# openMVG/openMVG

Measured on AMD Instinct MI355X. Metric: descriptor pairs/s (brute-force L2 2-NN + ratio matching), higher is better.
Workload: dtype i8 (int32 accumulate); 1 GPU; 1000 images x 2000 SIFT-like uint8x128 descriptors, exhaustive pairs (499500 image pairs, 499500 on rank 0), ratio 0.8; parallelism=pair-sharded x1, no collective

## Files before the change

openmvg_amd/csrc/mvgx_match.hip:

```cpp
#include <hip/hip_runtime.h>

#include <algorithm>
#include <atomic>
#include <climits>
#include <condition_variable>
#include <cstdint>
#include <cstdlib>
#include <cstring>
#include <functional>
#include <mutex>
#include <string>
#include <thread>
#include <vector>

#include "mvgx_common.h"

namespace {

using mvgx::set_error;

typedef int v4i __attribute__((ext_vector_type(4)));
typedef int v16i __attribute__((ext_vector_type(16)));

constexpr int kDim = 128;
constexpr int kTileRows = 32;
constexpr int kTileBytes = kTileRows * kDim;
constexpr int kWinTiles = 8;
constexpr int kWinRows = kWinTiles * kTileRows;
constexpr int kWaves = 4;
constexpr int kNQ = 4;
constexpr int kBlockQTiles = kWaves * kNQ;
constexpr int kRecQuads = 1 + kWaves;
constexpr int kStageBytes = kWinTiles * kTileBytes + kWinTiles * kTileRows * 4;
constexpr int kRPad = INT_MIN + 512;
constexpr int kCPad = -(1 << 27);
constexpr int kNegInit = -(1 << 28);
constexpr uint32_t kNoMatch = 0xFFFFFFFFu;
constexpr int kTailTiles = 16;

struct MatchParams {
  const int8_t* tiles;
  const int8_t* rows_slot;
  const int* rconst;
  const int* cinit;
  const int* qnorm;
  const uint32_t* perm;
  const uint32_t* rowpos;
  const uint8_t* rows_u8;
  const uint64_t* img_row_off;
  const uint32_t* img_tile_off;
  const uint32_t* img_n;
  const uint32_t* img_ntiles;
  const uint32_t* img_neven;
  const int8_t* qtiles;
  const int* qtnorm;
  const uint2* pairs;
  const uint2* work;
  const uint4* work8h;
  const uint4* work8;
  uint32_t n_work;
  uint32_t* best;
  int2* cd;
  uint32_t* count;
  uint32_t* errflag;
  uint32_t qstride;
  float ratio_sq;
};

__global__ __launch_bounds__(256) void row_norms_kernel(const uint8_t* __restrict__ rows,
                                                        const uint64_t* __restrict__ img_row_off,
                                                        const uint32_t* __restrict__ img_n, int* __restrict__ rownorm,
                                                        uint32_t* __restrict__ n_even) {
  const uint32_t img = blockIdx.y;
  const uint32_t n = img_n[img];
  const uint32_t r = blockIdx.x * blockDim.x + threadIdx.x;
  bool even = false;
  if (r < n) {
    const uint4* src = reinterpret_cast<const uint4*>(rows + (img_row_off[img] + r) * kDim);
    int nn = 0;
#pragma unroll
    for (int c = 0; c < 8; ++c) {
      uint4 v = src[c];
      const uint32_t w[4] = {v.x ^ 0x80808080u, v.y ^ 0x80808080u, v.z ^ 0x80808080u, v.w ^ 0x80808080u};
#pragma unroll
      for (int i = 0; i < 4; ++i) nn = __builtin_amdgcn_sdot4((int)w[i], (int)w[i], nn, false);
    }
    rownorm[img_row_off[img] + r] = nn;
    even = (nn & 1) == 0;
  }
  const unsigned long long m = __ballot(even);
  if ((threadIdx.x & 63) == 0 && m) atomicAdd(&n_even[img], (uint32_t)__popcll(m));
}

__device__ __host__ __forceinline__ int slot_row(int j, int h) { return (j >> 2) * 8 + h * 4 + (j & 3); }

__global__ __launch_bounds__(1024) void assign_slots_kernel(const uint64_t* __restrict__ img_row_off,
                                                            const uint32_t* __restrict__ img_tile_off,
                                                            const uint32_t* __restrict__ img_n,
                                                            const int* __restrict__ rownorm, uint32_t* __restrict__ rowpos,
                                                            uint32_t* __restrict__ perm, int* __restrict__ rconst,
                                                            int* __restrict__ cinit, int* __restrict__ qnorm) {
  __shared__ uint32_t s_cnt[16][2];
  __shared__ uint32_t s_base[2];
  const uint32_t img = blockIdx.x;
  const uint32_t n = img_n[img];
  const uint64_t row0 = img_row_off[img];
  const size_t slot0 = (size_t)img_tile_off[img] * kTileRows;
  const int lane = threadIdx.x & 63, wave = threadIdx.x >> 6;
  if (threadIdx.x < 2) s_base[threadIdx.x] = 0;
  __syncthreads();
  for (uint32_t c0 = 0; c0 < n; c0 += blockDim.x) {
    const uint32_t r = c0 + threadIdx.x;
    const bool valid = r < n;
    const int nn = valid ? rownorm[row0 + r] : 0;
    const int par = nn & 1;
    const unsigned long long m_even = __ballot(valid && par == 0), m_odd = __ballot(valid && par == 1);
    if (lane == 0) { s_cnt[wave][0] = (uint32_t)__popcll(m_even); s_cnt[wave][1] = (uint32_t)__popcll(m_odd); }
    __syncthreads();
    if (valid) {
      uint32_t rank = s_base[par];
      for (int w = 0; w < wave; ++w) rank += s_cnt[w][par];
      rank += (uint32_t)__popcll((par ? m_odd : m_even) & ((1ull << lane) - 1ull));
      const uint32_t t = rank >> 4;
      const uint32_t pos = t * kTileRows + (uint32_t)slot_row((int)(rank & 15u), par);
      rowpos[row0 + r] = pos;
      perm[slot0 + pos] = r;
      rconst[slot0 + pos] = -(nn << 8) - (int)((t % kWinTiles) * kTileRows + (pos & 31u));
      cinit[slot0 + pos] = -(nn >> 1);
      qnorm[slot0 + pos] = nn;
    }
    __syncthreads();
    if (threadIdx.x == 0) {
      uint32_t e = 0, o = 0;
      for (int w = 0; w < 16; ++w) { e += s_cnt[w][0]; o += s_cnt[w][1]; }
      s_base[0] += e; s_base[1] += o;
    }
    __syncthreads();
  }
}

__global__ __launch_bounds__(256) void build_tiles_kernel(const uint8_t* __restrict__ rows,
                                                          const uint64_t* __restrict__ img_row_off,
                                                          const uint32_t* __restrict__ img_tile_off,
                                                          const uint32_t* __restrict__ perm, int8_t* __restrict__ tiles,
                                                          int8_t* __restrict__ rows_slot) {
  const uint32_t img = blockIdx.y;
  const uint32_t ntiles_pad = img_tile_off[img + 1] - img_tile_off[img];
  const uint32_t t = blockIdx.x;
  if (t >= ntiles_pad) return;
  const uint32_t gt = img_tile_off[img] + t;
  const int c = threadIdx.x;
  const int s = c >> 6, lane = c & 63;
  const int m = lane & 31, h = lane >> 5;
  const uint32_t src_row = perm[(size_t)gt * kTileRows + m];
  uint4 v = make_uint4(0, 0, 0, 0);
  if (src_row != kNoMatch) {
    v = *reinterpret_cast<const uint4*>(rows + (img_row_off[img] + src_row) * kDim + (s * 2 + h) * 16);
    v.x ^= 0x80808080u; v.y ^= 0x80808080u; v.z ^= 0x80808080u; v.w ^= 0x80808080u;
  }
  *reinterpret_cast<uint4*>(tiles + (size_t)gt * kTileBytes + c * 16) = v;
  *reinterpret_cast<uint4*>(rows_slot + ((size_t)gt * kTileRows + m) * kDim + (s * 2 + h) * 16) = v;
}

__global__ __launch_bounds__(256) void build_qtiles_kernel(const uint8_t* __restrict__ rows,
                                                           const uint64_t* __restrict__ img_row_off,
                                                           const uint32_t* __restrict__ img_qtile_off,
                                                           const uint32_t* __restrict__ img_n,
                                                           const int* __restrict__ rownorm, int8_t* __restrict__ qtiles,
                                                           int* __restrict__ qtnorm) {
  const uint32_t img = blockIdx.y;
  const uint32_t t = blockIdx.x;
  if (t >= img_qtile_off[img + 1] - img_qtile_off[img]) return;
  const uint32_t gt = img_qtile_off[img] + t;
  const int c = threadIdx.x;
  const int s = c >> 6, lane = c & 63;
  const int m = lane & 31, h = lane >> 5;
  const uint32_t r = t * kTileRows + (uint32_t)m;
  const bool real = r < img_n[img];
  uint4 v = make_uint4(0, 0, 0, 0);
  if (real) {
    v = *reinterpret_cast<const uint4*>(rows + (img_row_off[img] + r) * kDim + (s * 2 + h) * 16);
    v.x ^= 0x80808080u; v.y ^= 0x80808080u; v.z ^= 0x80808080u; v.w ^= 0x80808080u;
  }
  *reinterpret_cast<uint4*>(qtiles + (size_t)gt * kTileBytes + c * 16) = v;
  if (c < kTileRows) qtnorm[(size_t)gt * kTileRows + m] = real ? rownorm[img_row_off[img] + r] : 0;
}

__global__ __launch_bounds__(256) void fill_i32_kernel(int* __restrict__ p, size_t n, int value) {
  const size_t i = (size_t)blockIdx.x * blockDim.x + threadIdx.x;
  if (i < n) p[i] = value;
}

__device__ __forceinline__ int med3i(int a, int b, int c) { return max(min(a, b), min(max(a, b), c)); }

__device__ __forceinline__ uint32_t xcd_remap(uint32_t b, uint32_t nwg) {
  const uint32_t q = nwg >> 3, r = nwg & 7u;
  const uint32_t xcd = b & 7u, pos = b >> 3;
  const uint32_t base = (xcd < r) ? xcd * (q + 1) : r * (q + 1) + (xcd - r) * q;
  return base + pos;
}

enum StageMode { kStageRegs = 1, kStageGlds = 2, kStageGldsAsm = 3 };


__device__ __forceinline__ void glds16_asm(const void* gsrc, unsigned lds_dst) {
  unsigned keep;
  asm volatile(
      "s_mov_b32 %0, m0\n\ts_mov_b32 m0, %2\n\ts_nop 0\n\tglobal_load_lds_dwordx4 %1, off\n\ts_mov_b32 m0, %0"
      : "=&s"(keep)
      : "v"(gsrc), "s"(lds_dst)
      : "memory");
}
__device__ __forceinline__ void glds4_asm(const void* gsrc, unsigned lds_dst) {
  unsigned keep;
  asm volatile(
      "s_mov_b32 %0, m0\n\ts_mov_b32 m0, %2\n\ts_nop 0\n\tglobal_load_lds_dword %1, off\n\ts_mov_b32 m0, %0"
      : "=&s"(keep)
      : "v"(gsrc), "s"(lds_dst)
      : "memory");
}
__device__ __forceinline__ void stage_window_glds_asm(char* buf, const int8_t* __restrict__ gtiles,
                                                      const int* __restrict__ grconst, int wave, int lane) {
  const unsigned lds0 = (unsigned)(size_t)(__attribute__((address_space(3))) char*)buf;
#pragma unroll
  for (int i = 0; i < kWinTiles; ++i) {
    const int off = i * kTileBytes + wave * 1024;
    glds16_asm(gtiles + off + lane * 16, __builtin_amdgcn_readfirstlane(lds0 + off));
  }
  glds4_asm(grconst + wave * 64 + lane, __builtin_amdgcn_readfirstlane(lds0 + kWinTiles * kTileBytes + wave * 256));
}

constexpr int kHalfTiles = kWinTiles / 2;
constexpr int kHalfStageBytes = kHalfTiles * kTileBytes + kHalfTiles * kTileRows * 4;
__device__ __forceinline__ void stage_half_glds_asm(char* buf, const int8_t* __restrict__ gtiles, const int* __restrict__ grconst, int wave, int lane) {
  const unsigned lds0 = (unsigned)(size_t)(__attribute__((address_space(3))) char*)buf;
#pragma unroll
  for (int i = 0; i < kHalfTiles; ++i) {
    const int off = i * kTileBytes + wave * 1024;
    glds16_asm(gtiles + off + lane * 16, __builtin_amdgcn_readfirstlane(lds0 + off));
  }
  if (wave < 2) glds4_asm(grconst + wave * 64 + lane, __builtin_amdgcn_readfirstlane(lds0 + kHalfTiles * kTileBytes + wave * 256));
}

__device__ __forceinline__ void stage_window_glds(char* buf, const int8_t* __restrict__ gtiles,
                                                  const int* __restrict__ grconst, int wave, int lane) {
#pragma unroll
  for (int i = 0; i < kWinTiles; ++i) {
    const int off = i * kTileBytes + wave * 1024;
    __builtin_amdgcn_global_load_lds((const void __attribute__((address_space(1)))*)(gtiles + off + lane * 16),
                                     (void __attribute__((address_space(3)))*)(buf + off), 16, 0, 0);
  }
  __builtin_amdgcn_global_load_lds(
      (const void __attribute__((address_space(1)))*)(grconst + wave * 64 + lane),
      (void __attribute__((address_space(3)))*)(buf + kWinTiles * kTileBytes + wave * 256), 4, 0, 0);
}

struct StageRegs {
  uint4 v[kWinTiles];
  int r;
};
__device__ __forceinline__ void stage_issue(StageRegs& sr, const int8_t* __restrict__ gtiles,
                                            const int* __restrict__ grconst, int wave, int lane) {
#pragma unroll
  for (int i = 0; i < kWinTiles; ++i)
    sr.v[i] = *reinterpret_cast<const uint4*>(gtiles + i * kTileBytes + wave * 1024 + lane * 16);
  sr.r = grconst[wave * 64 + lane];
}
__device__ __forceinline__ void stage_commit(char* buf, const StageRegs& sr, int wave, int lane) {
#pragma unroll
  for (int i = 0; i < kWinTiles; ++i)
    *reinterpret_cast<uint4*>(buf + i * kTileBytes + wave * 1024 + lane * 16) = sr.v[i];
  *reinterpret_cast<int*>(buf + kWinTiles * kTileBytes + wave * 256 + lane * 4) = sr.r;
}

struct Item32 {
  uint32_t pair, tileI0, tileJ0, ntJpad, qt0;
  int ntI, nwin;
};
__device__ __forceinline__ Item32 load_item32(const MatchParams& p, int wave, int lane, v4i (&b)[kNQ][4]) {
  const uint32_t w = xcd_remap(blockIdx.x, gridDim.x);
  const uint2 wk = p.work[w];
  const uint2 ij = p.pairs[wk.x];
  const uint32_t I = ij.x, J = ij.y;
  Item32 it;
  it.pair = wk.x;
  it.tileI0 = p.img_tile_off[I]; it.tileJ0 = p.img_tile_off[J];
  it.ntJpad = p.img_tile_off[J + 1] - it.tileJ0;
  it.ntI = (int)p.img_ntiles[I];
  it.nwin = (it.ntI + kWinTiles - 1) / kWinTiles;
  it.qt0 = wk.y + (uint32_t)wave * kNQ;
  const int8_t* qsrc = p.tiles + (size_t)(it.tileJ0 + it.qt0) * kTileBytes + lane * 16;
#pragma unroll
  for (int n = 0; n < kNQ; ++n)
#pragma unroll
    for (int s = 0; s < 4; ++s) b[n][s] = *reinterpret_cast<const v4i*>(qsrc + n * kTileBytes + s * 1024);
  return it;
}
__device__ __forceinline__ void pin_fragments32(v4i (&b)[kNQ][4]) {
#pragma unroll
  for (int n = 0; n < kNQ; ++n)
#pragma unroll
    for (int s = 0; s < 4; ++s) asm volatile("" : "+v"(b[n][s]));
}
template <int kMode>
__device__ __forceinline__ void stage_first(char* smem, StageRegs& sr, const int8_t* __restrict__ gI, const int* __restrict__ gC, int wave, int lane) {
  if constexpr (kMode == kStageGlds) {
    stage_window_glds(smem, gI, gC, wave, lane);
  } else if constexpr (kMode == kStageGldsAsm) {
    stage_window_glds_asm(smem, gI, gC, wave, lane);
  } else {
    stage_issue(sr, gI, gC, wave, lane);
    stage_commit(smem, sr, wave, lane);
  }
}
template <int kMode>
__device__ __forceinline__ void stage_next(char* nbuf, StageRegs& sr, const int8_t* __restrict__ gI, const int* __restrict__ gC, int win, int nwin,
                                           int wave, int lane) {
  if constexpr (kMode == kStageRegs) {
    const int wn = (win + 1 < nwin) ? win + 1 : win;
    stage_issue(sr, gI + (size_t)wn * kWinTiles * kTileBytes, gC + wn * kWinRows, wave, lane);
  } else if (win + 1 < nwin) {
    const int8_t* gt = gI + (size_t)(win + 1) * kWinTiles * kTileBytes;
    const int* gc = gC + (win + 1) * kWinRows;
    if constexpr (kMode == kStageGlds) stage_window_glds(nbuf, gt, gc, wave, lane);
    else stage_window_glds_asm(nbuf, gt, gc, wave, lane);
  }
}

template <int kMode>
__global__ __launch_bounds__(256, 2) void l2_top2_ratio_kernel(MatchParams p) {
  extern __shared__ __attribute__((aligned(16))) char smem[];

  const int lane = threadIdx.x & 63;
  const int wave = __builtin_amdgcn_readfirstlane(threadIdx.x >> 6);
  const int h = lane >> 5;

  v4i b[kNQ][4];
  const Item32 it = load_item32(p, wave, lane, b);
  const uint32_t tileI0 = it.tileI0, tileJ0 = it.tileJ0, ntJpad = it.ntJpad, qt0 = it.qt0;
  const int ntI = it.ntI, nwin = it.nwin;

  const int8_t* gI = p.tiles + (size_t)tileI0 * kTileBytes;
  const int* gR = p.rconst + (size_t)tileI0 * kTileRows;

  int G1[kNQ], G2[kNQ], Gi[kNQ];
#pragma unroll
  for (int n = 0; n < kNQ; ++n) { G1[n] = INT_MAX; G2[n] = INT_MAX; Gi[n] = 0; }

  StageRegs sr;
  stage_first<kMode>(smem, sr, gI, gR, wave, lane);
  pin_fragments32(b);

  for (int win = 0; win < nwin; ++win) {
    if constexpr (kMode == kStageGldsAsm) asm volatile("s_waitcnt vmcnt(0)" ::: "memory");
    __syncthreads();
    char* buf = smem + (win & 1) * kStageBytes;
    char* nbuf = smem + ((win + 1) & 1) * kStageBytes;
    stage_next<kMode>(nbuf, sr, gI, gR, win, nwin, wave, lane);

    int T1[kNQ], T2[kNQ];
#pragma unroll
    for (int n = 0; n < kNQ; ++n) { T1[n] = INT_MIN; T2[n] = INT_MIN; }

    const int nt = min(kWinTiles, ntI - win * kWinTiles);
    for (int t = 0; t < nt; ++t) {
      const char* tb = buf + t * kTileBytes + lane * 16;
      v4i a[4];
#pragma unroll
      for (int s = 0; s < 4; ++s) a[s] = *reinterpret_cast<const v4i*>(tb + s * 1024);
      const char* rb = buf + kWinTiles * kTileBytes + t * (kTileRows * 4) + h * 16;
      int R[16];
#pragma unroll
      for (int g = 0; g < 4; ++g) {
        const int4 rv = *reinterpret_cast<const int4*>(rb + g * 32);
        R[g * 4 + 0] = rv.x; R[g * 4 + 1] = rv.y; R[g * 4 + 2] = rv.z; R[g * 4 + 3] = rv.w;
      }
#pragma unroll
      for (int n = 0; n < kNQ; ++n) {
        v16i acc = {0, 0, 0, 0, 0, 0, 0, 0, 0, 0, 0, 0, 0, 0, 0, 0};
#pragma unroll
        for (int s = 0; s < 4; ++s) acc = __builtin_amdgcn_mfma_i32_32x32x32_i8(a[s], b[n][s], acc, 0, 0, 0);
        int t1 = T1[n], t2 = T2[n];
#pragma unroll
        for (int r = 0; r < 16; ++r) {
          const int T = (int)((unsigned)acc[r] << 9) + R[r];
          t2 = med3i(t1, t2, T);
          t1 = max(t1, T);
        }
        T1[n] = t1; T2[n] = t2;
      }
    }
    if constexpr (kMode == kStageRegs) stage_commit(nbuf, sr, wave, lane);
#pragma unroll
    for (int n = 0; n < kNQ; ++n) {
      const int k1 = -T1[n], k2 = -T2[n];
      const int wd1 = k1 >> 8, widx = (k1 & 255) + win * kWinRows, wd2 = k2 >> 8;
      const bool better = wd1 < G1[n];
      const int g2 = better ? min(G1[n], wd2) : min(G2[n], wd1);
      Gi[n] = better ? widx : Gi[n];
      G1[n] = better ? wd1 : G1[n];
      G2[n] = g2;
    }
  }

#pragma unroll
  for (int n = 0; n < kNQ; ++n) {
    const int P1 = __shfl_xor(G1[n], 32), P2 = __shfl_xor(G2[n], 32), Pi = __shfl_xor(Gi[n], 32);
    const bool better = P1 < G1[n];
    const int g2 = better ? min(G1[n], P2) : min(G2[n], P1);
    Gi[n] = better ? Pi : Gi[n];
    G1[n] = better ? P1 : G1[n];
    G2[n] = g2;
  }

#pragma unroll
  for (int n = 0; n < kNQ; ++n) {
    const uint32_t q = (qt0 + n) * kTileRows + (lane & 31);
    const bool inb = (lane < 32) && (qt0 + n < ntJpad);
    bool ok = false;
    if (inb) {
      const bool valid = p.perm[(size_t)tileJ0 * kTileRows + q] != kNoMatch;
      const int nq = p.qnorm[(size_t)tileJ0 * kTileRows + q];
      const int d0 = G1[n] + nq, d1 = G2[n] + nq;
      ok = valid && (__int2float_rn(d0) < __fmul_rn(p.ratio_sq, __int2float_rn(d1)));
      p.best[(size_t)it.pair * p.qstride + q] = ok ? p.perm[(size_t)tileI0 * kTileRows + (uint32_t)Gi[n]] : kNoMatch;
    }
    const unsigned long long m = __ballot(ok);
    if (lane == 0 && m) atomicAdd(&p.count[it.pair], (uint32_t)__popcll(m));
  }
}

__device__ __forceinline__ int max3i(int a, int b, int c) { return max(max(a, b), c); }

__device__ __forceinline__ void fold_window_max(int v, int& Q1, int& Q2, int& Qg, int win) {
  const bool better = v > Q1;
  Q2 = better ? Q1 : max(Q2, v);
  Qg = better ? win : Qg;
  Q1 = better ? v : Q1;
}
template <int kClasses>
__device__ __forceinline__ void fold_window(int (&TW)[kClasses], int (&TP)[kClasses], int& Q1, int& Q2, int& Qg, int win) {
  int v = TW[0];
#pragma unroll
  for (int c = 1; c < kClasses; ++c) v = max(v, TW[c]);
#pragma unroll
  for (int c = 0; c < kClasses; ++c) { TP[c] = max(TP[c], TW[c]); TW[c] = kNegInit; }
  fold_window_max(v, Q1, Q2, Qg, win);
}

enum FilterEpilogue { kEpiFold = 0, kEpiFoldOneCv = 1, kEpiPerChain = 2 };

template <int kMode, int kEpi = kEpiFold>
__global__ __launch_bounds__(256, 2) void l2_filter_kernel(MatchParams p) {
  extern __shared__ __attribute__((aligned(16))) char smem[];

  const int lane = threadIdx.x & 63;
  const int wave = __builtin_amdgcn_readfirstlane(threadIdx.x >> 6);
  const int h = lane >> 5;

  v4i b[kNQ][4];
  const Item32 it = load_item32(p, wave, lane, b);
  const uint32_t tileI0 = it.tileI0, tileJ0 = it.tileJ0, ntJpad = it.ntJpad, qt0 = it.qt0;
  const int ntI = it.ntI, nwin = it.nwin;

  const int8_t* gI = p.tiles + (size_t)tileI0 * kTileBytes;
  const int* gC = p.cinit + (size_t)tileI0 * kTileRows;

  constexpr bool kFold = kEpi != kEpiPerChain;
  constexpr bool kOneCv = kEpi == kEpiFoldOneCv;
  int TP[kNQ][8];
  int TW[kNQ][8];
  int Q1[kNQ], Q2[kNQ], Qg[kNQ];
#pragma unroll
  for (int n = 0; n < kNQ; ++n) {
#pragma unroll
    for (int s = 0; s < 8; ++s) { TP[n][s] = kNegInit; TW[n][s] = kNegInit; }
    Q1[n] = kNegInit; Q2[n] = kNegInit; Qg[n] = 0;
  }

  StageRegs sr;
  stage_first<kMode>(smem, sr, gI, gC, wave, lane);
  pin_fragments32(b);

  for (int win = 0; win < nwin; ++win) {
    if constexpr (kMode == kStageGldsAsm) asm volatile("s_waitcnt vmcnt(0)" ::: "memory");
    __syncthreads();
    char* buf = smem + (win & 1) * kStageBytes;
    char* nbuf = smem + ((win + 1) & 1) * kStageBytes;
    stage_next<kMode>(nbuf, sr, gI, gC, win, nwin, wave, lane);

    int TQ[kNQ];
#pragma unroll
    for (int n = 0; n < kNQ; ++n) TQ[n] = kNegInit;

    const int nt = min(kWinTiles, ntI - win * kWinTiles);
    const char* wb = buf + lane * 16;
    const char* wc = buf + kWinTiles * kTileBytes + h * 16;
    v4i a[4];
    v16i cv;
#pragma unroll
    for (int s = 0; s < 4; ++s) a[s] = *reinterpret_cast<const v4i*>(wb + s * 1024);
#pragma unroll
    for (int g = 0; g < 4; ++g) {
      const int4 c4 = *reinterpret_cast<const int4*>(wc + g * 32);
      cv[g * 4 + 0] = c4.x; cv[g * 4 + 1] = c4.y; cv[g * 4 + 2] = c4.z; cv[g * 4 + 3] = c4.w;
    }
    v16i accA, accB;
#pragma unroll
    for (int r = 0; r < 16; ++r) accB[r] = kNegInit;

#define MVGX_EPILOGUE(ACC, N)                                          \
  if constexpr (kFold) {                                               \
    _Pragma("unroll") for (int s = 0; s < 8; ++s)                      \
      TW[N][s] = max(max(TW[N][s], ACC[2 * s]), ACC[2 * s + 1]);       \
  } else {                                                             \
    int tq = TQ[N];                                                    \
    _Pragma("unroll") for (int s = 0; s < 8; ++s) {                    \
      TP[N][s] = max(max(TP[N][s], ACC[2 * s]), ACC[2 * s + 1]);       \
      tq = max(max(tq, ACC[2 * s + 1]), ACC[2 * s]);                   \
    }                                                                  \
    TQ[N] = tq;                                                        \
  }
#define MVGX_CHAIN(ACC, N, A, CV)                                                            \
  ACC = __builtin_amdgcn_mfma_i32_32x32x32_i8(A[0], b[N][0], CV, 0, 0, 0);                   \
  ACC = __builtin_amdgcn_mfma_i32_32x32x32_i8(A[1], b[N][1], ACC, 0, 0, 0);                  \
  ACC = __builtin_amdgcn_mfma_i32_32x32x32_i8(A[2], b[N][2], ACC, 0, 0, 0);                  \
  ACC = __builtin_amdgcn_mfma_i32_32x32x32_i8(A[3], b[N][3], ACC, 0, 0, 0);
#define MVGX_INTERLEAVE()                                                                    \
  _Pragma("unroll") for (int i_ = 0; i_ < 4; ++i_) {                                         \
    __builtin_amdgcn_sched_group_barrier(0x8, 1, 0);                                         \
    __builtin_amdgcn_sched_group_barrier(0x2, kFold ? 2 : 4, 0);                             \
  }
#define MVGX_LOAD_CINIT(CV, TN)                                                                    \
  _Pragma("unroll") for (int g = 0; g < 4; ++g) {                                                  \
    const int4 c4 = *reinterpret_cast<const int4*>(wc + (TN) * (kTileRows * 4) + g * 32);          \
    CV[g * 4 + 0] = c4.x; CV[g * 4 + 1] = c4.y; CV[g * 4 + 2] = c4.z; CV[g * 4 + 3] = c4.w;       \
  }
#define MVGX_TILE(A, CV, AN, CN, TN)                                                              \
  {                                                                                                \
    const int tn_ = (TN);                                                                          \
    MVGX_CHAIN(accA, 0, A, CV)                                                                     \
    _Pragma("unroll") for (int s = 0; s < 4; ++s)                                                  \
      AN[s] = *reinterpret_cast<const v4i*>(wb + tn_ * kTileBytes + s * 1024);                     \
    MVGX_EPILOGUE(accB, 3)                                                                         \
    MVGX_INTERLEAVE()                                                                              \
    MVGX_CHAIN(accB, 1, A, CV)                                                                     \
    if constexpr (!kOneCv) { MVGX_LOAD_CINIT(CN, tn_) }                                            \
    MVGX_EPILOGUE(accA, 0)                                                                         \
    MVGX_INTERLEAVE()                                                                              \
    MVGX_CHAIN(accA, 2, A, CV)                                                                     \
    MVGX_EPILOGUE(accB, 1)                                                                         \
    MVGX_INTERLEAVE()                                                                              \
    if constexpr (kOneCv) {   \
      accB = __builtin_amdgcn_mfma_i32_32x32x32_i8(A[0], b[3][0], CV, 0, 0, 0);                   \
      MVGX_LOAD_CINIT(CV, tn_)                                                                     \
      accB = __builtin_amdgcn_mfma_i32_32x32x32_i8(A[1], b[3][1], accB, 0, 0, 0);                 \
      accB = __builtin_amdgcn_mfma_i32_32x32x32_i8(A[2], b[3][2], accB, 0, 0, 0);                 \
      accB = __builtin_amdgcn_mfma_i32_32x32x32_i8(A[3], b[3][3], accB, 0, 0, 0);                 \
    } else {                                                                                       \
      MVGX_CHAIN(accB, 3, A, CV)                                                                   \
    }                                                                                              \
    MVGX_EPILOGUE(accA, 2)                                                                         \
    MVGX_INTERLEAVE()                                                                              \
  }
    v4i an[4];
    v16i cn;
    int t = 0;
    if constexpr (kOneCv) {
      for (; t + 1 < nt; t += 2) {
        MVGX_TILE(a, cv, an, cv, t + 1)
        MVGX_TILE(an, cv, a, cv, min(t + 2, nt - 1))
      }
      if (t < nt) MVGX_TILE(a, cv, an, cv, t)
    } else {
      for (; t + 1 < nt; t += 2) {
        MVGX_TILE(a, cv, an, cn, t + 1)
        MVGX_TILE(an, cn, a, cv, min(t + 2, nt - 1))
      }
      if (t < nt) MVGX_TILE(a, cv, an, cn, t)
    }
    MVGX_EPILOGUE(accB, 3)
#undef MVGX_EPILOGUE
#undef MVGX_CHAIN
#undef MVGX_LOAD_CINIT
#undef MVGX_TILE
#undef MVGX_INTERLEAVE
    if constexpr (kMode == kStageRegs) stage_commit(nbuf, sr, wave, lane);
#pragma unroll
    for (int n = 0; n < kNQ; ++n) {
      if constexpr (kFold) fold_window<8>(TW[n], TP[n], Q1[n], Q2[n], Qg[n], win);
      else fold_window_max(TQ[n], Q1[n], Q2[n], Qg[n], win);
    }
  }

#pragma unroll
  for (int n = 0; n < kNQ; ++n) {
    int p1 = kNegInit, p2 = kNegInit, ps = 0;
#pragma unroll
    for (int s = 0; s < 8; ++s) {
      const int v = TP[n][s];
      const bool better = v > p1;
      p2 = better ? p1 : max(p2, v);
      ps = better ? s : ps;
      p1 = better ? v : p1;
    }
    const int w1 = 2 * p1 - h, w2p = 2 * p2 - h, w2q = 2 * Q2[n] - h;
    const int o1 = __shfl_xor(w1, 32), o2p = __shfl_xor(w2p, 32), o2q = __shfl_xor(w2q, 32);
    const int os = __shfl_xor(ps, 32), og = __shfl_xor(Qg[n], 32);
    const bool mine = w1 > o1;
    const int W1 = mine ? w1 : o1;
    const int V2 = mine ? max3i(w2p, w2q, o1) : max3i(o2p, o2q, w1);
    const int s1 = mine ? ps : os, g1 = mine ? Qg[n] : og, hw = mine ? h : (h ^ 1);

    const uint32_t q = (qt0 + n) * kTileRows + (lane & 31);
    if (lane < 32 && qt0 + n < ntJpad) {
      const bool valid = p.perm[(size_t)tileJ0 * kTileRows + q] != kNoMatch;
      const int nq = p.qnorm[(size_t)tileJ0 * kTileRows + q];
      const int d0 = nq - W1, d1ub = nq - V2;
      const bool cand = valid && (__int2float_rn(d0) < __fmul_rn(p.ratio_sq, __int2float_rn(d1ub)));
      const size_t o = (size_t)it.pair * p.qstride + q;
      p.best[o] = cand ? ((uint32_t)s1 | ((uint32_t)hw << 3) | ((uint32_t)g1 << 4)) : kNoMatch;
      if (cand) p.cd[o] = make_int2(d0, d1ub);
    }
  }
}

constexpr int kNB16 = 2 * kNQ;

#define MVGX_GROUP16(ACC, N0, A, CV)                                                                       \
  _Pragma("unroll") for (int i_ = 0; i_ < 4; ++i_)                                                          \
    ACC[i_] = __builtin_amdgcn_mfma_i32_16x16x64_i8(A[0], b[(N0) + i_][0], CV, 0, 0, 0);                    \
  _Pragma("unroll") for (int i_ = 0; i_ < 4; ++i_)                                                          \
    ACC[i_] = __builtin_amdgcn_mfma_i32_16x16x64_i8(A[1], b[(N0) + i_][1], ACC[i_], 0, 0, 0);
#define MVGX_EPI16(ACC, N0, BLK)                                                                            \
  _Pragma("unroll") for (int i_ = 0; i_ < 4; ++i_) {                                                        \
    TW[(N0) + i_][2 * (BLK)] = max(max(TW[(N0) + i_][2 * (BLK)], ACC[i_][0]), ACC[i_][1]);                  \
    TW[(N0) + i_][2 * (BLK) + 1] = max(max(TW[(N0) + i_][2 * (BLK) + 1], ACC[i_][2]), ACC[i_][3]);          \
  }
#define MVGX_MIX16(NDS)                                                                                     \
  _Pragma("unroll") for (int i_ = 0; i_ < 8; ++i_) {                                                        \
    __builtin_amdgcn_sched_group_barrier(0x8, 1, 0);                                                        \
    __builtin_amdgcn_sched_group_barrier(0x2, 1, 0);                                                        \
    if (i_ < (NDS)) __builtin_amdgcn_sched_group_barrier(0x100, 1, 0);                                      \
  }

#define MVGX_FINISH16(N, INB, VALID)                                                                                                      \
  {                                                                                                                                       \
    int p1 = kNegInit, p2 = kNegInit, pc = 0;                                                \
    _Pragma("unroll") for (int c = 0; c < 4; ++c) {                                                                                       \
      const int v = TP[N][c];                                                                                                             \
      const bool better = v > p1;                                                                                                         \
      p2 = better ? p1 : max(p2, v);                                                                                                      \
      pc = better ? c : pc;                                                                                                               \
      p1 = better ? v : p1;                                                                                                               \
    }                                                                                                                                     \
                          \
    int W1 = 2 * p1 - par, V2 = max(2 * p2 - par, 2 * Q2[N] - par);                                                                       \
    int code = (4 * (pc >> 1) + 2 * (g4 >> 1) + (pc & 1)) | (par << 3) | (Qg[N] << 4);    \
        \
            \
                                                                       \
    _Pragma("unroll") for (int x = 16; x <= 32; x <<= 1) {                                                                                \
      const int o1 = __shfl_xor(W1, x), o2 = __shfl_xor(V2, x), oc = __shfl_xor(code, x);                                                 \
      const bool mine = W1 > o1;                                                                                                          \
      V2 = mine ? max(V2, o1) : max(o2, W1);                                                                                              \
      code = mine ? code : oc;                                                                                                            \
      W1 = mine ? W1 : o1;                                                                                                                \
    }                                                                                                                                     \
    const uint32_t q = (qt0 + (uint32_t)((N) >> 1)) * kTileRows + (uint32_t)((N) & 1) * 16 + (uint32_t)(lane & 15);                       \
    if (lane < 16 && (INB)) {                                                                                                             \
      const int nq = qn[N];                                                                                                               \
      const int d0 = nq - W1, d1ub = nq - V2;                                                                                             \
      const bool cand = (VALID) && (__int2float_rn(d0) < __fmul_rn(p.ratio_sq, __int2float_rn(d1ub)));                                    \
      const size_t o = (size_t)pair * p.qstride + q;                                                                                      \
      p.best[o] = cand ? (uint32_t)code : kNoMatch;                                                                                       \
      if (cand) p.cd[o] = make_int2(d0, d1ub);                                                                                            \
    }                                                                                                                                     \
  }

__global__ __launch_bounds__(256, 2) void l2_filter16_kernel(MatchParams p) {
  extern __shared__ __attribute__((aligned(16))) char smem[];

  const int lane = threadIdx.x & 63;
  const int wave = __builtin_amdgcn_readfirstlane(threadIdx.x >> 6);
  const int g4 = lane >> 4, par = g4 & 1;

  const uint32_t w = xcd_remap(blockIdx.x, gridDim.x);
  const uint4* rec = p.work8 + (size_t)kRecQuads * w;
  const uint4 wsh = rec[0], wun = rec[1 + wave];
  const uint32_t tileI0 = wsh.x;
  const int ntI = (int)wsh.y;
  const uint32_t pair = wun.x, tileJ0 = wun.y, qt0 = wun.z;
  const uint32_t nJ = wun.w;
  const int nwin = (ntI + kWinTiles - 1) / kWinTiles;

  const int lane_chunk = ((lane >> 5) * 64 + ((lane >> 4) & 1) * 32 + (lane & 15)) * 16;
  v4i b[kNB16][2];
  {
    const int8_t* qsrc = p.qtiles + (size_t)(tileJ0 + qt0) * kTileBytes + lane_chunk;
#pragma unroll
    for (int n = 0; n < kNB16; ++n)
#pragma unroll
      for (int ks = 0; ks < 2; ++ks) b[n][ks] = *reinterpret_cast<const v4i*>(qsrc + (n >> 1) * kTileBytes + (n & 1) * 256 + ks * 2048);
  }

  const int8_t* gI = p.tiles + (size_t)tileI0 * kTileBytes;
  const int* gC = p.cinit + (size_t)tileI0 * kTileRows;

  int qn[kNB16];
#pragma unroll
  for (int n = 0; n < kNB16; ++n) {
    const uint32_t q = (qt0 + (uint32_t)(n >> 1)) * kTileRows + (uint32_t)(n & 1) * 16 + (uint32_t)(lane & 15);
    qn[n] = (lane < 16 && q < nJ) ? p.qtnorm[(size_t)tileJ0 * kTileRows + q] : 0;
  }

  int TP[kNB16][4];
  int TW[kNB16][4];
  int Q1[kNB16], Q2[kNB16], Qg[kNB16];
#pragma unroll
  for (int n = 0; n < kNB16; ++n) {
#pragma unroll
    for (int c = 0; c < 4; ++c) { TP[n][c] = kNegInit; TW[n][c] = kNegInit; }
    Q1[n] = kNegInit; Q2[n] = kNegInit; Qg[n] = 0;
  }

  stage_window_glds_asm(smem, gI, gC, wave, lane);
#pragma unroll
  for (int n = 0; n < kNB16; ++n) {
#pragma unroll
    for (int ks = 0; ks < 2; ++ks) asm volatile("" : "+v"(b[n][ks]));
    asm volatile("" : "+v"(qn[n]));
  }

  for (int win = 0; win < nwin; ++win) {
    asm volatile("s_waitcnt vmcnt(0)" ::: "memory");
    __syncthreads();
    char* buf = smem + (win & 1) * kStageBytes;
    char* nbuf = smem + ((win + 1) & 1) * kStageBytes;
    if (win + 1 < nwin)
      stage_window_glds_asm(nbuf, gI + (size_t)(win + 1) * kWinTiles * kTileBytes, gC + (win + 1) * kWinRows, wave, lane);

    const int nt = min(kWinTiles, ntI - win * kWinTiles);
    const char* wb = buf + lane_chunk;
    const char* wc = buf + kWinTiles * kTileBytes + g4 * 16;
    v4i accA[4], accB[4];
#pragma unroll
    for (int i = 0; i < 4; ++i) accB[i] = v4i{kNegInit, kNegInit, kNegInit, kNegInit};

#define MVGX_BLOCK16(A, CV, AN, CN, BLK, NEXT_OFF, NEXT_COFF)                                               \
  {                                                                                                         \
    MVGX_GROUP16(accA, 0, A, CV)                                                                            \
    AN[0] = *reinterpret_cast<const v4i*>(wb + (NEXT_OFF));                                                 \
    AN[1] = *reinterpret_cast<const v4i*>(wb + (NEXT_OFF) + 2048);                                          \
    MVGX_EPI16(accB, 4, 1 - (BLK))                                                                          \
    MVGX_MIX16(2)                                                                                           \
    MVGX_GROUP16(accB, 4, A, CV)                                                                            \
    CN = *reinterpret_cast<const v4i*>(wc + (NEXT_COFF));                                                   \
    MVGX_EPI16(accA, 0, BLK)                                                                                \
    MVGX_MIX16(1)                                                                                           \
  }
    v4i a0[2], a1[2], c0, c1;
    a0[0] = *reinterpret_cast<const v4i*>(wb);
    a0[1] = *reinterpret_cast<const v4i*>(wb + 2048);
    c0 = *reinterpret_cast<const v4i*>(wc);
    __builtin_amdgcn_s_setprio(3);
    for (int t = 0; t < nt; ++t) {
      const int tn = min(t + 1, nt - 1);
      MVGX_BLOCK16(a0, c0, a1, c1, 0, t * kTileBytes + 256, t * (kTileRows * 4) + 64)
      MVGX_BLOCK16(a1, c1, a0, c0, 1, tn * kTileBytes, tn * (kTileRows * 4))
    }
    MVGX_EPI16(accB, 4, 1)
    __builtin_amdgcn_s_setprio(0);
#undef MVGX_BLOCK16
#pragma unroll
    for (int n = 0; n < kNB16; ++n) fold_window<4>(TW[n], TP[n], Q1[n], Q2[n], Qg[n], win);
  }

#pragma unroll
  for (int n = 0; n < kNB16; ++n) MVGX_FINISH16(n, q < nJ, true)
}

constexpr int kNQh = 2;
constexpr int kNBh = 2 * kNQh;
constexpr int kBlockQTilesH = kWaves * kNQh;
__global__ __launch_bounds__(256, 3) void l2_filter16h_kernel(MatchParams p) {
  extern __shared__ __attribute__((aligned(16))) char smem[];

  const int lane = threadIdx.x & 63;
  const int wave = __builtin_amdgcn_readfirstlane(threadIdx.x >> 6);
  const int g4 = lane >> 4, par = g4 & 1;

  const uint32_t w = xcd_remap(blockIdx.x, gridDim.x);
  const uint4 wr0 = p.work8h[2 * (size_t)w], wr1 = p.work8h[2 * (size_t)w + 1];
  const uint32_t pair = wr0.x;
  const uint32_t tileI0 = wr0.z, tileJ0 = wr0.w;
  const uint32_t ntJpad = wr1.y;
  const int ntI = (int)wr1.x;
  const int nhalf = (ntI + kHalfTiles - 1) / kHalfTiles;
  const uint32_t qt0 = wr0.y + (uint32_t)wave * kNQh;

  const int lane_chunk = ((lane >> 5) * 64 + ((lane >> 4) & 1) * 32 + (lane & 15)) * 16;
  v4i b[kNBh][2];
  {
    const int8_t* qsrc = p.tiles + (size_t)(tileJ0 + qt0) * kTileBytes + lane_chunk;
#pragma unroll
    for (int n = 0; n < kNBh; ++n)
#pragma unroll
      for (int ks = 0; ks < 2; ++ks) b[n][ks] = *reinterpret_cast<const v4i*>(qsrc + (n >> 1) * kTileBytes + (n & 1) * 256 + ks * 2048);
  }
  const int8_t* gI = p.tiles + (size_t)tileI0 * kTileBytes;
  const int* gC = p.cinit + (size_t)tileI0 * kTileRows;

  uint32_t qperm[kNBh];
  int qn[kNBh];
#pragma unroll
  for (int n = 0; n < kNBh; ++n) {
    const bool inb = lane < 16 && qt0 + (uint32_t)(n >> 1) < ntJpad;
    const size_t qs = (size_t)tileJ0 * kTileRows + (qt0 + (uint32_t)(n >> 1)) * kTileRows + (uint32_t)(n & 1) * 16 + (uint32_t)(lane & 15);
    qperm[n] = inb ? p.perm[qs] : kNoMatch;
    qn[n] = inb ? p.qnorm[qs] : 0;
  }

  int TP[kNBh][4], TW[kNBh][4], Q1[kNBh], Q2[kNBh], Qg[kNBh];
#pragma unroll
  for (int n = 0; n < kNBh; ++n) {
#pragma unroll
    for (int c = 0; c < 4; ++c) { TP[n][c] = kNegInit; TW[n][c] = kNegInit; }
    Q1[n] = kNegInit; Q2[n] = kNegInit; Qg[n] = 0;
  }

  stage_half_glds_asm(smem, gI, gC, wave, lane);
#pragma unroll
  for (int n = 0; n < kNBh; ++n) {
#pragma unroll
    for (int ks = 0; ks < 2; ++ks) asm volatile("" : "+v"(b[n][ks]));
    asm volatile("" : "+v"(qperm[n]), "+v"(qn[n]));
  }

  for (int hw = 0; hw < nhalf; ++hw) {
    asm volatile("s_waitcnt vmcnt(0)" ::: "memory");
    __syncthreads();
    char* buf = smem + (hw & 1) * kHalfStageBytes;
    char* nbuf = smem + ((hw + 1) & 1) * kHalfStageBytes;
    if (hw + 1 < nhalf)
      stage_half_glds_asm(nbuf, gI + (size_t)(hw + 1) * kHalfTiles * kTileBytes, gC + (hw + 1) * kHalfTiles * kTileRows, wave, lane);

    const int nt = min(kHalfTiles, ntI - hw * kHalfTiles);
    const char* wb = buf + lane_chunk;
    const char* wc = buf + kHalfTiles * kTileBytes + g4 * 16;
    v4i accA[4], accB[4];
#pragma unroll
    for (int i = 0; i < 4; ++i) accB[i] = v4i{kNegInit, kNegInit, kNegInit, kNegInit};
    v4i a0[2], a1[2], c0, c1;
    a0[0] = *reinterpret_cast<const v4i*>(wb);
    a0[1] = *reinterpret_cast<const v4i*>(wb + 2048);
    c0 = *reinterpret_cast<const v4i*>(wc);
    for (int t = 0; t < nt; ++t) {
      const int tn = min(t + 1, nt - 1);
      MVGX_GROUP16(accA, 0, a0, c0)
      a1[0] = *reinterpret_cast<const v4i*>(wb + t * kTileBytes + 256);
      a1[1] = *reinterpret_cast<const v4i*>(wb + t * kTileBytes + 256 + 2048);
      c1 = *reinterpret_cast<const v4i*>(wc + t * (kTileRows * 4) + 64);
      MVGX_EPI16(accB, 0, 1)
      MVGX_MIX16(3)
      MVGX_GROUP16(accB, 0, a1, c1)
      a0[0] = *reinterpret_cast<const v4i*>(wb + tn * kTileBytes);
      a0[1] = *reinterpret_cast<const v4i*>(wb + tn * kTileBytes + 2048);
      c0 = *reinterpret_cast<const v4i*>(wc + tn * (kTileRows * 4));
      MVGX_EPI16(accA, 0, 0)
      MVGX_MIX16(3)
    }
    MVGX_EPI16(accB, 0, 1)
    if ((hw & 1) || hw + 1 == nhalf) {
#pragma unroll
      for (int n = 0; n < kNBh; ++n) fold_window<4>(TW[n], TP[n], Q1[n], Q2[n], Qg[n], hw >> 1);
    }
  }

#pragma unroll
  for (int n = 0; n < kNBh; ++n) MVGX_FINISH16(n, qt0 + (uint32_t)(n >> 1) < ntJpad, qperm[n] != kNoMatch)
}
#undef MVGX_FINISH16
#undef MVGX_GROUP16
#undef MVGX_EPI16
#undef MVGX_MIX16

__device__ __forceinline__ int sum8_dpp(int v) {
  v += __builtin_amdgcn_update_dpp(0, v, 0xB1, 0xF, 0xF, true);
  v += __builtin_amdgcn_update_dpp(0, v, 0x4E, 0xF, 0xF, true);
  v += __builtin_amdgcn_update_dpp(0, v, 0x141, 0xF, 0xF, true);
  return v;
}
__device__ __forceinline__ int min16_dpp(int v) {
  v = min(v, __builtin_amdgcn_update_dpp(INT_MAX, v, 0xB1, 0xF, 0xF, false));
  v = min(v, __builtin_amdgcn_update_dpp(INT_MAX, v, 0x4E, 0xF, 0xF, false));
  v = min(v, __builtin_amdgcn_update_dpp(INT_MAX, v, 0x141, 0xF, 0xF, false));
  v = min(v, __builtin_amdgcn_update_dpp(INT_MAX, v, 0x140, 0xF, 0xF, false));
  return v;
}

template <bool kWaveUnits>
__global__ __launch_bounds__(256) void l2_verify_kernel(MatchParams p) {
  const int lane = threadIdx.x & 63;
  const int wave = threadIdx.x >> 6;
  uint32_t pair, qt0, I, tileI0, tileJ0, qend;
  const uint8_t* rowsJ = nullptr;
  if constexpr (kWaveUnits) {
    const uint4* rec = p.work8 + (size_t)kRecQuads * blockIdx.x;
    const uint4 wun = rec[1 + __builtin_amdgcn_readfirstlane(wave)];
    pair = wun.x; tileJ0 = wun.y; qt0 = wun.z; qend = wun.w;
    tileI0 = rec[0].x;
    const uint2 ij = p.pairs[pair];
    I = ij.x;
    rowsJ = p.rows_u8 + p.img_row_off[ij.y] * kDim;
  } else {
    const uint2 wk = p.work[blockIdx.x];
    const uint2 ij = p.pairs[wk.x];
    pair = wk.x; qt0 = wk.y + (uint32_t)wave * kNQ;
    I = ij.x;
    tileI0 = p.img_tile_off[I]; tileJ0 = p.img_tile_off[ij.y];
    qend = (p.img_tile_off[ij.y + 1] - tileJ0) * kTileRows;
  }
  const uint32_t nEvenI = p.img_neven[I], nOddI = p.img_n[I] - nEvenI;
  const int l16 = lane & 15, sub = lane >> 4;
  uint32_t accepted = 0;
  for (int part = 0; part < 2; ++part) {
    const uint32_t q0 = qt0 * kTileRows + (uint32_t)part * 64;
    const uint32_t q = q0 + lane;
    const bool inb = q < qend;
    const uint32_t code = inb ? p.best[(size_t)pair * p.qstride + q] : kNoMatch;
    unsigned long long todo = __ballot(code != kNoMatch);
    while (todo) {
      unsigned long long m = todo;
      for (int i = 0; i < sub; ++i) m &= m - 1;
      const bool active = m != 0;
      const int src = active ? __builtin_ctzll(m) : 0;
      for (int i = 0; i < 4; ++i) todo &= todo - 1;
      const uint32_t cc = (uint32_t)__shfl((int)code, src);
      const uint32_t qs = q0 + (uint32_t)src;
      const int s1 = cc & 7, hw = (cc >> 3) & 1, g1 = (int)(cc >> 4);
      const int piece = l16 & 7, rsel = l16 >> 3;
      const int mrow = slot_row(2 * s1 + rsel, hw);
      const size_t slot0 = (size_t)tileI0 * kTileRows + (active ? (size_t)g1 * kWinTiles * kTileRows + mrow : 0);
      const size_t slotQ = (size_t)tileJ0 * kTileRows + (active ? qs : 0);
      const size_t o = (size_t)pair * p.qstride + (active ? qs : 0);
      const uint32_t tt = (uint32_t)g1 * kWinTiles + (uint32_t)piece;
      const size_t slotI = active ? slot0 + (size_t)piece * kTileRows : slot0;
      const bool valid = active && (tt * 16u + (uint32_t)(2 * s1 + rsel)) < (hw ? nOddI : nEvenI);
      int4 va[8];
#pragma unroll
      for (int c = 0; c < 8; ++c)
        va[c] = *reinterpret_cast<const int4*>(p.rows_slot + (slot0 + (active ? (size_t)c * kTileRows : 0)) * kDim + piece * 16);
      int4 vb;
      if constexpr (kWaveUnits) {
        vb = *reinterpret_cast<const int4*>(rowsJ + (size_t)(active ? qs : 0) * kDim + piece * 16);
        vb.x ^= (int)0x80808080u; vb.y ^= (int)0x80808080u; vb.z ^= (int)0x80808080u; vb.w ^= (int)0x80808080u;
      } else {
        vb = *reinterpret_cast<const int4*>(p.rows_slot + slotQ * kDim + piece * 16);
      }
      const int2 f = p.cd[o];
      const int f_d0 = f.x, f_d1 = f.y;
      int nb = __builtin_amdgcn_sdot4(vb.x, vb.x, 0, false);
      nb = __builtin_amdgcn_sdot4(vb.y, vb.y, nb, false);
      nb = __builtin_amdgcn_sdot4(vb.z, vb.z, nb, false);
      nb = __builtin_amdgcn_sdot4(vb.w, vb.w, nb, false);
      nb = sum8_dpp(nb);
      int dot = 0, na = 0;
#pragma unroll
      for (int c = 0; c < 8; ++c) {
        int part = __builtin_amdgcn_sdot4(va[c].x, vb.x, 0, false);
        part = __builtin_amdgcn_sdot4(va[c].y, vb.y, part, false);
        part = __builtin_amdgcn_sdot4(va[c].z, vb.z, part, false);
        part = __builtin_amdgcn_sdot4(va[c].w, vb.w, part, false);
        part = sum8_dpp(part);
        dot = (c == piece) ? part : dot;
        int sq = __builtin_amdgcn_sdot4(va[c].x, va[c].x, 0, false);
        sq = __builtin_amdgcn_sdot4(va[c].y, va[c].y, sq, false);
        sq = __builtin_amdgcn_sdot4(va[c].z, va[c].z, sq, false);
        sq = __builtin_amdgcn_sdot4(va[c].w, va[c].w, sq, false);
        sq = sum8_dpp(sq);
        na = (c == piece) ? sq : na;
      }
      const int d = valid ? na + nb - 2 * dot : INT_MAX;
      const int key = min16_dpp(valid ? ((d << 4) | l16) : INT_MAX);
      const int wl = key & 15, dbest = key >> 4;
      const int second = min16_dpp((l16 == wl) ? INT_MAX : d);
      bool ok = false;
      if (active && l16 == wl) {
        if (key == INT_MAX || dbest != f_d0) atomicAdd(p.errflag, 1u);
        const int d1 = min(f_d1, second);
        ok = __int2float_rn(dbest) < __fmul_rn(p.ratio_sq, __int2float_rn(d1));
        p.best[o] = ok ? p.perm[slotI] : kNoMatch;
      }
      accepted += (uint32_t)__popcll(__ballot(ok));
    }
  }
  if (lane == 0 && accepted) atomicAdd(&p.count[pair], accepted);
}

__global__ __launch_bounds__(256) void count_candidates_kernel(const uint32_t* __restrict__ best, size_t n,
                                                               uint32_t* __restrict__ counter) {
  __shared__ uint32_t s_sum;
  if (threadIdx.x == 0) s_sum = 0;
  __syncthreads();
  uint32_t c = 0;
  const size_t base = (size_t)blockIdx.x * 16384;
  for (int k = 0; k < 64; ++k) {
    const size_t i = base + (size_t)k * 256 + threadIdx.x;
    if (i < n && best[i] != kNoMatch) ++c;
  }
  const unsigned long long m = __ballot(c != 0);
  (void)m;
  for (int off = 32; off > 0; off >>= 1) c += __shfl_down(c, off);
  if ((threadIdx.x & 63) == 0 && c) atomicAdd(&s_sum, c);
  __syncthreads();
  if (threadIdx.x == 0 && s_sum) atomicAdd(counter, s_sum);
}

__global__ __launch_bounds__(256) void count_candidates_units_kernel(MatchParams p, uint32_t* __restrict__ counter) {
  __shared__ uint32_t s_sum;
  if (threadIdx.x == 0) s_sum = 0;
  __syncthreads();
  const int lane = threadIdx.x & 63, wave = threadIdx.x >> 6;
  const uint4 wun = p.work8[(size_t)kRecQuads * blockIdx.x + 1 + wave];
  uint32_t c = 0;
  for (int part = 0; part < 2; ++part) {
    const uint32_t q = wun.z * kTileRows + (uint32_t)part * 64 + (uint32_t)lane;
    const bool cand = q < wun.w && p.best[(size_t)wun.x * p.qstride + q] != kNoMatch;
    c += (uint32_t)__popcll(__ballot(cand));
  }
  if (lane == 0 && c) atomicAdd(&s_sum, c);
  __syncthreads();
  if (threadIdx.x == 0 && s_sum) atomicAdd(counter, s_sum);
}

__global__ __launch_bounds__(256) void l2_top2_ratio_naive_kernel(MatchParams p) {
  const uint2 wk = p.work[blockIdx.x];
  const uint2 ij = p.pairs[wk.x];
  const uint32_t I = ij.x, J = ij.y;
  const uint32_t nI = p.img_n[I], nJ = p.img_n[J];
  const uint8_t* rowsI = p.rows_u8 + p.img_row_off[I] * kDim;
  const uint8_t* rowsJ = p.rows_u8 + p.img_row_off[J] * kDim;
  for (uint32_t q = wk.y * kTileRows + threadIdx.x; q < min(nJ, (wk.y + kBlockQTiles) * kTileRows);
       q += blockDim.x) {
    uint32_t qv[32];
#pragma unroll
    for (int k = 0; k < 32; ++k) qv[k] = reinterpret_cast<const uint32_t*>(rowsJ + (size_t)q * kDim)[k];
    int d0 = INT_MAX, d1 = INT_MAX;
    uint32_t i0 = 0;
    for (uint32_t i = 0; i < nI; ++i) {
      const uint32_t* dbr = reinterpret_cast<const uint32_t*>(rowsI + (size_t)i * kDim);
      int d = 0;
#pragma unroll
      for (int k = 0; k < 32; ++k) {
        const uint32_t x = qv[k], y = dbr[k];
#pragma unroll
        for (int bb = 0; bb < 4; ++bb) {
          const int df = (int)((x >> (8 * bb)) & 0xFF) - (int)((y >> (8 * bb)) & 0xFF);
          d += df * df;
        }
      }
      if (d < d0) { d1 = d0; d0 = d; i0 = i; }
      else if (d < d1) { d1 = d; }
    }
    const bool ok = __int2float_rn(d0) < __fmul_rn(p.ratio_sq, __int2float_rn(d1));
    p.best[(size_t)wk.x * p.qstride + p.rowpos[p.img_row_off[J] + q]] = ok ? i0 : kNoMatch;
    if (ok) atomicAdd(&p.count[wk.x], 1u);
  }
}

__global__ __launch_bounds__(1024) void scan_counts_kernel(const uint32_t* __restrict__ count, uint32_t n,
                                                           uint32_t* __restrict__ offsets ) {
  __shared__ uint32_t s_part[1024];
  const uint32_t per = (n + 1023) / 1024;
  const uint32_t lo = min(n, threadIdx.x * per), hi = min(n, lo + per);
  uint32_t sum = 0;
  for (uint32_t i = lo; i < hi; ++i) sum += count[i];
  s_part[threadIdx.x] = sum;
  __syncthreads();
  for (uint32_t d = 1; d < 1024; d <<= 1) {
    const uint32_t v = (threadIdx.x >= d) ? s_part[threadIdx.x - d] : 0;
    __syncthreads();
// ... 935 lines not shown
```

Baseline: 9786 billion descriptor pairs/s.

## Unroll full-window tile loop, peel first-tile epilogue, use SGPR-base LDS loads

The l2_filter16 kernel now fully unrolls the tile loop when a window is full (kWinTiles tiles). It peels the first tiles so the running max is initialised by assignment instead of max against a -inf sentinel, and the last tile skips its redundant prefetch. Global-to-LDS staging moves to a scalar-base plus per-lane offset form, so per-tile 64-bit vector address arithmetic goes away. The window fold and final top-2 selection use med3-based updates. Together these aim to cut VALU and address overhead in the inner MFMA loop, at the cost of larger code and a separate path for partial windows.

```diff
diff --git a/openmvg_amd/csrc/mvgx_match.hip b/openmvg_amd/csrc/mvgx_match.hip
--- a/openmvg_amd/csrc/mvgx_match.hip
+++ b/openmvg_amd/csrc/mvgx_match.hip
@@ -230,6 +230,32 @@
   glds4_asm(grconst + wave * 64 + lane, __builtin_amdgcn_readfirstlane(lds0 + kWinTiles * kTileBytes + wave * 256));
 }
 
+#define MVGX_GLDS_SBASE 1
+__device__ __forceinline__ void glds16_sasm(const void* sbase, unsigned voff, unsigned lds_dst) {
+  unsigned keep;
+  asm volatile(
+      "s_mov_b32 %0, m0\n\ts_mov_b32 m0, %3\n\ts_nop 0\n\tglobal_load_lds_dwordx4 %1, %2\n\ts_mov_b32 m0, %0"
+      : "=&s"(keep)
+      : "v"(voff), "s"(sbase), "s"(lds_dst)
+      : "memory");
+}
+__device__ __forceinline__ void glds4_sasm(const void* sbase, unsigned voff, unsigned lds_dst) {
+  unsigned keep;
+  asm volatile(
+      "s_mov_b32 %0, m0\n\ts_mov_b32 m0, %3\n\ts_nop 0\n\tglobal_load_lds_dword %1, %2\n\ts_mov_b32 m0, %0"
+      : "=&s"(keep)
+      : "v"(voff), "s"(sbase), "s"(lds_dst)
+      : "memory");
+}
+__device__ __forceinline__ void stage_window_glds_sasm(char* buf, const int8_t* __restrict__ gtiles, const int* __restrict__ grconst,
+                                                       unsigned voff16, unsigned voff4, int wave) {
+  const unsigned lds0 = (unsigned)(size_t)(__attribute__((address_space(3))) char*)buf;
+#pragma unroll
+  for (int i = 0; i < kWinTiles; ++i)
+    glds16_sasm(gtiles + i * kTileBytes, voff16, __builtin_amdgcn_readfirstlane(lds0 + i * kTileBytes + wave * 1024));
+  glds4_sasm(grconst, voff4, __builtin_amdgcn_readfirstlane(lds0 + kWinTiles * kTileBytes + wave * 256));
+}
+
 constexpr int kHalfTiles = kWinTiles / 2;
 constexpr int kHalfStageBytes = kHalfTiles * kTileBytes + kHalfTiles * kTileRows * 4;
 __device__ __forceinline__ void stage_half_glds_asm(char* buf, const int8_t* __restrict__ gtiles, const int* __restrict__ grconst, int wave, int lane) {
@@ -678,6 +704,68 @@
     }                                                                                                                                     \
   }
 
+#define MVGX_EPI16_FIRST(ACC, N0, BLK)                                                                      \
+  _Pragma("unroll") for (int i_ = 0; i_ < 4; ++i_) {                                                        \
+    TW[(N0) + i_][2 * (BLK)] = max(ACC[i_][0], ACC[i_][1]);                                                 \
+    TW[(N0) + i_][2 * (BLK) + 1] = max(ACC[i_][2], ACC[i_][3]);                                             \
+  }
+#define MVGX_EPI16_NONE(ACC, N0, BLK)
+#define MVGX_MIX16_NOEPI(NDS)                                                                               \
+  _Pragma("unroll") for (int i_ = 0; i_ < 8; ++i_) {                                                        \
+    __builtin_amdgcn_sched_group_barrier(0x8, 1, 0);                                                        \
+    if (i_ < (NDS)) __builtin_amdgcn_sched_group_barrier(0x100, 1, 0);                                      \
+  }
+
+__device__ __forceinline__ void stage_window16(char* buf, const int8_t* __restrict__ gtiles, const int* __restrict__ grconst,
+                                               unsigned voff16, unsigned voff4, int wave, int lane) {
+#ifdef MVGX_GLDS_SBASE
+  stage_window_glds_sasm(buf, gtiles, grconst, voff16, voff4, wave);
+#else
+  stage_window_glds_asm(buf, gtiles, grconst, wave, lane);
+#endif
+}
+
+__device__ __forceinline__ void fold_window16(const int (&TW)[4], int (&TP)[4], int& Q1, int& Q2, int& Qg, int win) {
+  const int v = max(max3i(TW[0], TW[1], TW[2]), TW[3]);
+#pragma unroll
+  for (int c = 0; c < 4; ++c) TP[c] = max(TP[c], TW[c]);
+  Qg = v > Q1 ? win : Qg;
+  Q2 = med3i(Q1, v, Q2);
+  asm volatile("" : "+v"(Q1));
+  Q1 = max(Q1, v);
+}
+
+#define MVGX_FINISH16_MED3(N, INB, VALID)                                                                                                 \
+  {                                                                                                                                       \
+    int p1 = kNegInit, p2 = kNegInit, pc = 0;                                                \
+    _Pragma("unroll") for (int c = 0; c < 4; ++c) {                                                                                       \
+      const int v = TP[N][c];                                                                                                             \
+      pc = v > p1 ? c : pc;                                                                                                               \
+      p2 = med3i(p1, v, p2);                                                                                                              \
+      p1 = max(p1, v);                                                                                                                    \
+    }                                                                                                                                     \
+                          \
+    int W1 = 2 * p1 - par, V2 = max(2 * p2 - par, 2 * Q2[N] - par);                                                                       \
+    int code = (4 * (pc >> 1) + 2 * (g4 >> 1) + (pc & 1)) | (par << 3) | (Qg[N] << 4);    \
+                                                  \
+    _Pragma("unroll") for (int x = 16; x <= 32; x <<= 1) {                                                                                \
+      const int o1 = __shfl_xor(W1, x), o2 = __shfl_xor(V2, x), oc = __shfl_xor(code, x);                                                 \
+      const bool mine = W1 > o1;                                                                                                          \
+      V2 = mine ? max(V2, o1) : max(o2, W1);                                                                                              \
+      code = mine ? code : oc;                                                                                                            \
+      W1 = mine ? W1 : o1;                                                                                                                \
+    }                                                                                                                                     \
+    const uint32_t q = (qt0 + (uint32_t)((N) >> 1)) * kTileRows + (uint32_t)((N) & 1) * 16 + (uint32_t)(lane & 15);                       \
+    if (lane < 16 && (INB)) {                                                                                                             \
+      const int nq = qn[N];                                                                                                               \
+      const int d0 = nq - W1, d1ub = nq - V2;                                                                                             \
+      const bool cand = (VALID) && (__int2float_rn(d0) < __fmul_rn(p.ratio_sq, __int2float_rn(d1ub)));                                    \
+      const size_t o = (size_t)pair * p.qstride + q;                                                                                      \
+      p.best[o] = cand ? (uint32_t)code : kNoMatch;                                                                                       \
+      if (cand) p.cd[o] = make_int2(d0, d1ub);                                                                                            \
+    }                                                                                                                                     \
+  }
+
 __global__ __launch_bounds__(256, 2) void l2_filter16_kernel(MatchParams p) {
   extern __shared__ __attribute__((aligned(16))) char smem[];
 
@@ -720,11 +808,12 @@
 #pragma unroll
   for (int n = 0; n < kNB16; ++n) {
 #pragma unroll
-    for (int c = 0; c < 4; ++c) { TP[n][c] = kNegInit; TW[n][c] = kNegInit; }
+    for (int c = 0; c < 4; ++c) TP[n][c] = kNegInit;
     Q1[n] = kNegInit; Q2[n] = kNegInit; Qg[n] = 0;
   }
 
-  stage_window_glds_asm(smem, gI, gC, wave, lane);
+  const unsigned voff16 = (unsigned)(lane * 16 + wave * 1024), voff4 = (unsigned)(lane * 4 + wave * 256);
+  stage_window16(smem, gI, gC, voff16, voff4, wave, lane);
 #pragma unroll
   for (int n = 0; n < kNB16; ++n) {
 #pragma unroll
@@ -738,46 +827,70 @@
     char* buf = smem + (win & 1) * kStageBytes;
     char* nbuf = smem + ((win + 1) & 1) * kStageBytes;
     if (win + 1 < nwin)
-      stage_window_glds_asm(nbuf, gI + (size_t)(win + 1) * kWinTiles * kTileBytes, gC + (win + 1) * kWinRows, wave, lane);
+      stage_window16(nbuf, gI + (size_t)(win + 1) * kWinTiles * kTileBytes, gC + (win + 1) * kWinRows, voff16, voff4, wave, lane);
 
     const int nt = min(kWinTiles, ntI - win * kWinTiles);
     const char* wb = buf + lane_chunk;
     const char* wc = buf + kWinTiles * kTileBytes + g4 * 16;
     v4i accA[4], accB[4];
-#pragma unroll
-    for (int i = 0; i < 4; ++i) accB[i] = v4i{kNegInit, kNegInit, kNegInit, kNegInit};
-
-#define MVGX_BLOCK16(A, CV, AN, CN, BLK, NEXT_OFF, NEXT_COFF)                                               \
+
+#define MVGX_BLOCK16(A, CV, AN, CN, BLK, LD, NEXT_OFF, NEXT_COFF, EPI_B, MIX_B, EPI_A)                      \
   {                                                                                                         \
     MVGX_GROUP16(accA, 0, A, CV)                                                                            \
-    AN[0] = *reinterpret_cast<const v4i*>(wb + (NEXT_OFF));                                                 \
-    AN[1] = *reinterpret_cast<const v4i*>(wb + (NEXT_OFF) + 2048);                                          \
-    MVGX_EPI16(accB, 4, 1 - (BLK))                                                                          \
-    MVGX_MIX16(2)                                                                                           \
+    if (LD) {                                                                                               \
+      AN[0] = *reinterpret_cast<const v4i*>(wb + (NEXT_OFF));                                               \
+      AN[1] = *reinterpret_cast<const v4i*>(wb + (NEXT_OFF) + 2048);                                        \
+    }                                                                                                       \
+    EPI_B(accB, 4, 1 - (BLK))                                                                               \
+    MIX_B((LD) ? 2 : 0)                                                                                     \
     MVGX_GROUP16(accB, 4, A, CV)                                                                            \
-    CN = *reinterpret_cast<const v4i*>(wc + (NEXT_COFF));                                                   \
-    MVGX_EPI16(accA, 0, BLK)                                                                                \
-    MVGX_MIX16(1)                                                                                           \
-  }
+    if (LD) CN = *reinterpret_cast<const v4i*>(wc + (NEXT_COFF));                                           \
+    EPI_A(accA, 0, BLK)                                                                                     \
+    MVGX_MIX16((LD) ? 1 : 0)                                                                                \
+  }
+#define MVGX_TILE16(T)                                                                                                                       \
+  MVGX_BLOCK16(a0, c0, a1, c1, 0, true, (T) * kTileBytes + 256, (T) * (kTileRows * 4) + 64, MVGX_EPI16, MVGX_MIX16, MVGX_EPI16)              \
+  MVGX_BLOCK16(a1, c1, a0, c0, 1, true, ((T) + 1) * kTileBytes, ((T) + 1) * (kTileRows * 4), MVGX_EPI16, MVGX_MIX16, MVGX_EPI16)                \
+  MVGX_TILE16_END
+#define MVGX_TILE16_END __builtin_amdgcn_sched_barrier(0);
     v4i a0[2], a1[2], c0, c1;
     a0[0] = *reinterpret_cast<const v4i*>(wb);
     a0[1] = *reinterpret_cast<const v4i*>(wb + 2048);
     c0 = *reinterpret_cast<const v4i*>(wc);
     __builtin_amdgcn_s_setprio(3);
-    for (int t = 0; t < nt; ++t) {
-      const int tn = min(t + 1, nt - 1);
-      MVGX_BLOCK16(a0, c0, a1, c1, 0, t * kTileBytes + 256, t * (kTileRows * 4) + 64)
-      MVGX_BLOCK16(a1, c1, a0, c0, 1, tn * kTileBytes, tn * (kTileRows * 4))
+    if (nt == kWinTiles) {
+      MVGX_BLOCK16(a0, c0, a1, c1, 0, true, 256, 64, MVGX_EPI16_NONE, MVGX_MIX16_NOEPI, MVGX_EPI16_FIRST)
+      MVGX_BLOCK16(a1, c1, a0, c0, 1, true, kTileBytes, kTileRows * 4, MVGX_EPI16_FIRST, MVGX_MIX16, MVGX_EPI16_FIRST)
+      MVGX_TILE16_END
+      MVGX_BLOCK16(a0, c0, a1, c1, 0, true, kTileBytes + 256, kTileRows * 4 + 64, MVGX_EPI16_FIRST, MVGX_MIX16, MVGX_EPI16)
+      MVGX_BLOCK16(a1, c1, a0, c0, 1, true, 2 * kTileBytes, 2 * (kTileRows * 4), MVGX_EPI16, MVGX_MIX16, MVGX_EPI16)
+      MVGX_TILE16_END
+      MVGX_TILE16(2) MVGX_TILE16(3) MVGX_TILE16(4) MVGX_TILE16(5) MVGX_TILE16(6)
+      MVGX_BLOCK16(a0, c0, a1, c1, 0, true, 7 * kTileBytes + 256, 7 * (kTileRows * 4) + 64, MVGX_EPI16, MVGX_MIX16, MVGX_EPI16)
+      MVGX_BLOCK16(a1, c1, a0, c0, 1, false, 0, 0, MVGX_EPI16, MVGX_MIX16, MVGX_EPI16)
+    } else {
+#pragma unroll
+      for (int n = 4; n < kNB16; ++n) { TW[n][2] = kNegInit; TW[n][3] = kNegInit; }
+      const int t1 = min(1, nt - 1);
+      MVGX_BLOCK16(a0, c0, a1, c1, 0, true, 256, 64, MVGX_EPI16_NONE, MVGX_MIX16_NOEPI, MVGX_EPI16_FIRST)
+      MVGX_BLOCK16(a1, c1, a0, c0, 1, true, t1 * kTileBytes, t1 * (kTileRows * 4), MVGX_EPI16_FIRST, MVGX_MIX16, MVGX_EPI16_FIRST)
+      for (int t = 1; t < nt; ++t) {
+        const int tn = min(t + 1, nt - 1);
+        MVGX_BLOCK16(a0, c0, a1, c1, 0, true, t * kTileBytes + 256, t * (kTileRows * 4) + 64, MVGX_EPI16, MVGX_MIX16, MVGX_EPI16)
+        MVGX_BLOCK16(a1, c1, a0, c0, 1, true, tn * kTileBytes, tn * (kTileRows * 4), MVGX_EPI16, MVGX_MIX16, MVGX_EPI16)
+      }
     }
     MVGX_EPI16(accB, 4, 1)
     __builtin_amdgcn_s_setprio(0);
+#undef MVGX_TILE16
+#undef MVGX_TILE16_END
 #undef MVGX_BLOCK16
 #pragma unroll
-    for (int n = 0; n < kNB16; ++n) fold_window<4>(TW[n], TP[n], Q1[n], Q2[n], Qg[n], win);
-  }
-
-#pragma unroll
-  for (int n = 0; n < kNB16; ++n) MVGX_FINISH16(n, q < nJ, true)
+    for (int n = 0; n < kNB16; ++n) fold_window16(TW[n], TP[n], Q1[n], Q2[n], Qg[n], win);
+  }
+
+#pragma unroll
+  for (int n = 0; n < kNB16; ++n) MVGX_FINISH16_MED3(n, q < nJ, true)
 }
 
 constexpr int kNQh = 2;
```

Measured after the change: 10100 billion descriptor pairs/s, median of 6. 3.3% higher.
